# SRainGit/CAE-LO

Measured on AMD Instinct MI355X. Metric: KITTI frames/sec end-to-end (keypts+desc+match+RANSAC), higher is better.
Workload: dtype f32

## Files before the change

cae-lo_amd/csrc/ransac.hip:

```cpp
#include "caelo_internal.h"
#include "caelo_rigid.h"

__device__ inline float residual(const float *R, const float *T, float ax, float ay, float az, float bx, float by, float bz) {
    const float px = __fadd_rn(__fadd_rn(__fadd_rn(__fmul_rn(R[0], bx), __fmul_rn(R[1], by)), __fmul_rn(R[2], bz)), T[0]);
    const float py = __fadd_rn(__fadd_rn(__fadd_rn(__fmul_rn(R[3], bx), __fmul_rn(R[4], by)), __fmul_rn(R[5], bz)), T[1]);
    const float pz = __fadd_rn(__fadd_rn(__fadd_rn(__fmul_rn(R[6], bx), __fmul_rn(R[7], by)), __fmul_rn(R[8], bz)), T[2]);
    const float dx = __fsub_rn(ax, px), dy = __fsub_rn(ay, py), dz = __fsub_rn(az, pz);
    return sqrtf(__fadd_rn(__fadd_rn(__fmul_rn(dx, dx), __fmul_rn(dy, dy)), __fmul_rn(dz, dz)));
}

__global__ void __launch_bounds__(256) k_solve_rt(const float *p0, const float *p1, int n, float *R, float *T, int *credible) {
    __shared__ double red[4][RIGID_TERMS];
    const int tid = threadIdx.x;
    RigidSums sums;
    for (int i = tid; i < n; i += 256) {
        const float *u = p0 + 3 * (size_t)i, *v = p1 + 3 * (size_t)i;
        sums.add(u[0], u[1], u[2], v[0], v[1], v[2]);
    }
    sums.reduce_wave(red, tid & 63, tid >> 6);
    __syncthreads();
    if (tid == 0) {
        double s[RIGID_TERMS];
        for (int t = 0; t < RIGID_TERMS; ++t) s[t] = RigidSums::combine(red, 4, t);
        const int cred = rigid_from_sums(s, R, T);
// ... 131 lines not shown
    }
#pragma unroll
    for (int i = 0; i < 3; ++i)
#pragma unroll
        for (int j = 0; j < 3; ++j) {
            double h = 0;
#pragma unroll
            for (int q = 0; q < 4; ++q) h += (double)c1[q][i] * (double)c0[q][j];
            H[3 * i + j] = h;
        }
    rigid_from_H<false>(H, m0, m1, R, T);
}

#define RB_G 9.5367431640625e-7f
struct HypBound {
    float a, b;
    int kind;
};
__device__ inline void hypothesis_bound(const Sample4 &s, HypBound &hb) {
    const double *H = s.H;
    const double C0 = H[4] * H[8] - H[5] * H[7], C1 = H[5] * H[6] - H[3] * H[8], C2 = H[3] * H[7] - H[4] * H[6];
    const double C3 = H[2] * H[7] - H[1] * H[8], C4 = H[0] * H[8] - H[2] * H[6], C5 = H[1] * H[6] - H[0] * H[7];
    const double C6 = H[1] * H[5] - H[2] * H[4], C7 = H[2] * H[3] - H[0] * H[5], C8 = H[0] * H[4] - H[1] * H[3];
    const double det = H[0] * C0 + H[1] * C1 + H[2] * C2;
    double I1 = 0.0;
#pragma unroll
    for (int i = 0; i < 9; ++i) I1 += H[i] * H[i];
    const double I2 = C0 * C0 + C1 * C1 + C2 * C2 + C3 * C3 + C4 * C4 + C5 * C5 + C6 * C6 + C7 * C7 + C8 * C8;
    float sumCA = 0.f;
    const float aC[9] = {(float)fabs(C0), (float)fabs(C1), (float)fabs(C2), (float)fabs(C3), (float)fabs(C4), (float)fabs(C5), (float)fabs(C6), (float)fabs(C7), (float)fabs(C8)};
#pragma unroll
    for (int i = 0; i < 3; ++i)
#pragma unroll
        for (int j = 0; j < 3; ++j) {
            float t = 0.f;
#pragma unroll
            for (int q = 0; q < 4; ++q) t += fabsf(s.c1[q][i]) * fabsf(s.c0[q][j]);
            sumCA += aC[3 * i + j] * t;
        }
    hb.kind = 0;
    hb.a = 0.f;
    hb.b = 0.f;
    if (!(I2 > 1e-10 * I1 * I1) || !(I1 > 0.0)) { hb.kind = 2; return; }
    const double kappa = 1.41421356237309515 * I1 / sqrt(I2);
    if (fabs(det) <= 64.0 * 5.9604644775390625e-8 * 1.001 * (double)sumCA) hb.kind = 1;
    if (det * det <= 1e-24 * I1 * I2) hb.kind = 1;
    const double nm0 = sqrt(s.m0[0] * s.m0[0] + s.m0[1] * s.m0[1] + s.m0[2] * s.m0[2]);
    const double nm1 = sqrt(s.m1[0] * s.m1[0] + s.m1[1] * s.m1[1] + s.m1[2] * s.m1[2]);
    hb.a = (float)(1.0001 * (double)RB_G * ((2.0 + kappa) * nm1 + nm0));
    hb.b = (float)(1.0001 * (double)RB_G * (2.0 + kappa));
}

#define RE_WAVES 4
#define RE_LDS_PAIRS 1024

__device__ inline void lane_agreement(const float R[9], const float T[3], int lane, int32_t *faults) {
    if (!faults) return;
    unsigned int diff = 0;
#pragma unroll
    for (int q = 0; q < 9; ++q) diff |= __float_as_uint(R[q]) ^ (unsigned int)__builtin_amdgcn_readfirstlane((int)__float_as_uint(R[q]));
#pragma unroll
    for (int q = 0; q < 3; ++q) diff |= __float_as_uint(T[q]) ^ (unsigned int)__builtin_amdgcn_readfirstlane((int)__float_as_uint(T[q]));
    if (__ballot(diff != 0) != 0ull && lane == 0) atomicAdd(faults, 1);
}

__device__ inline int hypothesis_count(const float *P0, int l0, const int64_t *pidx, const float *P1, int l1, int N, const double *r4,
                                       float thr, int lane, int32_t *faults) {
    float R[9], T[3];
    sample_hypothesis(P0, l0, pidx, P1, l1, N, r4, R, T);
    lane_agreement(R, T, lane, faults);
    int cnt = 0;
    for (int i = lane; i < ((N + 63) & ~63); i += 64) {
        bool in = false;
        if (i < N) {
            const float *a = P0 + (size_t)l0 * (pidx ? pidx[i] : i);
            const float *b = P1 + (size_t)l1 * i;
            in = residual(R, T, a[0], a[1], a[2], b[0], b[1], b[2]) < thr;
        }
        cnt += __popcll(__ballot(in));
    }
    return cnt;
}

#define RH_PER_WAVE 4
template <bool CERT>
__device__ __forceinline__ void four_hypotheses(const float *sP0, const float *sP1, int N, const double *rnd, int trial0, float thr, int lane,
                                       int32_t *faults, int32_t *counts, const float2 *sN = nullptr, caelo_ransac_cert *cert = nullptr,
                                       int level = 0) {
    const int mine = min(trial0 + (lane & (RH_PER_WAVE - 1)), CAELO_RANSAC_MAX_TRIALS - 1);
    float R[9], T[3];
    HypBound hb = {0.f, 0.f, 0};
    if (CERT) {
        Sample4 smp;
        sample4(sP0, 3, nullptr, sP1, 3, N, rnd + (size_t)mine * 4, smp);
        hypothesis_bound(smp, hb);
        if (lane < RH_PER_WAVE && trial0 + lane < CAELO_RANSAC_MAX_TRIALS)
#pragma unroll
            for (int q = 0; q < 4; ++q) (level ? cert->idx_up[level - 1] : cert->idx)[trial0 + lane][q] = smp.idx[q];
        rigid_from_H<false>(smp.H, smp.m0, smp.m1, R, T);
    } else {
        sample_hypothesis(sP0, 3, nullptr, sP1, 3, N, rnd + (size_t)mine * 4, R, T);
    }
    if (faults) {
        unsigned int hsh = 0;
#pragma unroll
        for (int q = 0; q < 9; ++q) hsh = hsh * 0x9E3779B1u + __float_as_uint(R[q]);
#pragma unroll
        for (int q = 0; q < 3; ++q) hsh = hsh * 0x9E3779B1u + __float_as_uint(T[q]);
        const bool bad = hsh != (unsigned int)__shfl_xor((int)hsh, 4) || hsh != (unsigned int)__shfl_xor((int)hsh, 16) ||
                         hsh != (unsigned int)__shfl_xor((int)hsh, 32);
        if (__ballot(bad) != 0ull && lane == 0) atomicAdd(faults, 1);
    }
    float Rs[RH_PER_WAVE][9], Ts[RH_PER_WAVE][3];
#pragma unroll
    for (int h = 0; h < RH_PER_WAVE; ++h) {
#pragma unroll
        for (int q = 0; q < 9; ++q) Rs[h][q] = __int_as_float(__builtin_amdgcn_readlane(__float_as_int(R[q]), h));
#pragma unroll
        for (int q = 0; q < 3; ++q) Ts[h][q] = __int_as_float(__builtin_amdgcn_readlane(__float_as_int(T[q]), h));
    }
    int cnt[RH_PER_WAVE] = {0, 0, 0, 0};
    if (!CERT) {
        for (int i = lane; i < ((N + 63) & ~63); i += 64) {
            const bool live = i < N;
            const int ii = live ? i : 0;
            const float ax = sP0[3 * ii], ay = sP0[3 * ii + 1], az = sP0[3 * ii + 2];
            const float bx = sP1[3 * ii], by = sP1[3 * ii + 1], bz = sP1[3 * ii + 2];
#pragma unroll
            for (int h = 0; h < RH_PER_WAVE; ++h) {
                const bool in = live && residual(Rs[h], Ts[h], ax, ay, az, bx, by, bz) < thr;
                cnt[h] += __popcll(__ballot(in));
            }
        }
    } else {
        float as[RH_PER_WAVE], bs[RH_PER_WAVE];
        int kinds[RH_PER_WAVE];
#pragma unroll
        for (int h = 0; h < RH_PER_WAVE; ++h) {
            as[h] = thr + __int_as_float(__builtin_amdgcn_readlane(__float_as_int(hb.a), h));
            bs[h] = __int_as_float(__builtin_amdgcn_readlane(__float_as_int(hb.b), h));
            kinds[h] = __builtin_amdgcn_readlane(hb.kind, h);
        }
        int hi[RH_PER_WAVE] = {0, 0, 0, 0};
        for (int i = lane; i < ((N + 63) & ~63); i += 64) {
            const bool live = i < N;
            const int ii = live ? i : 0;
            const float ax = sP0[3 * ii], ay = sP0[3 * ii + 1], az = sP0[3 * ii + 2];
            const float bx = sP1[3 * ii], by = sP1[3 * ii + 1], bz = sP1[3 * ii + 2];
            const float2 nn = sN[ii];
#pragma unroll
            for (int h = 0; h < RH_PER_WAVE; ++h) {
                const float r = residual(Rs[h], Ts[h], ax, ay, az, bx, by, bz);
                cnt[h] += __popcll(__ballot(live && r < thr));
                hi[h] += __popcll(__ballot(live && r < as[h] + fmaf(bs[h], nn.x, nn.y)));
            }
        }
        if ((kinds[0] | kinds[1] | kinds[2] | kinds[3]) & 1) {
            float Ra[9], Ta[3], Rb[9], Tb[3];
            bool two;
            {
                Sample4 smp;
                sample4(sP0, 3, nullptr, sP1, 3, N, rnd + (size_t)mine * 4, smp);
                two = rigid_two_candidates(smp.H, smp.m0, smp.m1, Ra, Ta, Rb, Tb);
            }
            int ha[RH_PER_WAVE] = {0, 0, 0, 0};
#pragma unroll 1
            for (int h = 0; h < RH_PER_WAVE; ++h) {
                if (kinds[h] != 1) continue;
                if (!__builtin_amdgcn_readlane((int)two, h)) { ha[h] = N; continue; }
                float Ras[9], Tas[3], Rbs[9], Tbs[3];
#pragma unroll
                for (int q = 0; q < 9; ++q) {
                    Ras[q] = __int_as_float(__builtin_amdgcn_readlane(__float_as_int(Ra[q]), h));
                    Rbs[q] = __int_as_float(__builtin_amdgcn_readlane(__float_as_int(Rb[q]), h));
                }
#pragma unroll
                for (int q = 0; q < 3; ++q) {
                    Tas[q] = __int_as_float(__builtin_amdgcn_readlane(__float_as_int(Ta[q]), h));
                    Tbs[q] = __int_as_float(__builtin_amdgcn_readlane(__float_as_int(Tb[q]), h));
                }
                int na = 0, nb = 0;
                for (int i = lane; i < ((N + 63) & ~63); i += 64) {
                    const bool live = i < N;
                    const int ii = live ? i : 0;
                    const float ax = sP0[3 * ii], ay = sP0[3 * ii + 1], az = sP0[3 * ii + 2];
                    const float bx = sP1[3 * ii], by = sP1[3 * ii + 1], bz = sP1[3 * ii + 2];
                    const float2 nn = sN[ii];
                    const float lim = as[h] + fmaf(bs[h], nn.x, nn.y);
                    na += __popcll(__ballot(live && residual(Ras, Tas, ax, ay, az, bx, by, bz) < lim));
                    nb += __popcll(__ballot(live && residual(Rbs, Tbs, ax, ay, az, bx, by, bz) < lim));
                }
                ha[h] = max(na, nb);
            }
#pragma unroll
            for (int h = 0; h < RH_PER_WAVE; ++h)
                if (kinds[h] == 1) hi[h] = max(hi[h], ha[h]);
        }
#pragma unroll
        for (int h = 0; h < RH_PER_WAVE; ++h)
            if (kinds[h] == 2) hi[h] = N;
        if (lane < RH_PER_WAVE && trial0 + lane < CAELO_RANSAC_MAX_TRIALS)
            (level ? cert->hi_up[level - 1] : cert->hi)[trial0 + lane] = lane == 0 ? hi[0] : (lane == 1 ? hi[1] : (lane == 2 ? hi[2] : hi[3]));
    }
    if (lane < RH_PER_WAVE && trial0 + lane < CAELO_RANSAC_MAX_TRIALS)
        counts[trial0 + lane] = lane == 0 ? cnt[0] : (lane == 1 ? cnt[1] : (lane == 2 ? cnt[2] : cnt[3]));
}

template <class PS>
static __device__ __forceinline__ void ransac_hyp_body(const PS &ps, int ld0, int ld1, int64_t k1_max) {
    const auto &P = pair_of(ps, blockIdx.z);
    const float *__restrict__ pc0 = P.pc0, *__restrict__ pc1 = P.pc1;
    const int64_t *__restrict__ pair_idx = P.pair_idx;
    RansacWs *ws = (RansacWs *)P.ws_ransac;
    __shared__ float sP0[RE_LDS_PAIRS * 3], sP1[RE_LDS_PAIRS * 3];
    __shared__ float2 sN[RE_LDS_PAIRS];
    caelo_ransac_cert *cert = P.cert;
    const int N = (P.n0 && *P.n0 <= 0) ? 0 : (P.n1 ? min(max(*P.n1, 0), (int)k1_max) : (int)k1_max);
    const int tid = threadIdx.x, lane = tid & 63, wave = tid >> 6;
    const bool in_lds = N <= RE_LDS_PAIRS;
    if (in_lds) {
        for (int i = tid; i < N; i += 64 * RE_WAVES) {
            const float *a = pc0 + (size_t)ld0 * pair_idx[i];
            const float *b = pc1 + (size_t)ld1 * i;
            const float a0 = a[0], a1 = a[1], a2 = a[2], b0 = b[0], b1 = b[1], b2 = b[2];
            sP0[3 * i] = a0; sP0[3 * i + 1] = a1; sP0[3 * i + 2] = a2;
            sP1[3 * i] = b0; sP1[3 * i + 1] = b1; sP1[3 * i + 2] = b2;
            if (cert) sN[i] = make_float2(1.0001f * sqrtf(b0 * b0 + b1 * b1 + b2 * b2), 1.0001f * RB_G * sqrtf(a0 * a0 + a1 * a1 + a2 * a2));
        }
    }
    __syncthreads();
    if (cert && blockIdx.x == 0 && tid == 0) cert->levels_up = 0;
    if (cert && P.cert_only && blockIdx.x == 0) {
        if (in_lds) {
            float *d0 = &cert->p0[0][0], *d1 = &cert->p1[0][0];
            for (int i = tid; i < 3 * N; i += 64 * RE_WAVES) { d0[i] = sP0[i]; d1[i] = sP1[i]; }
        }
        if (tid == 0) {
            cert->n_pairs = N;
            cert->flags = in_lds ? 0 : CAELO_CERT_NO_BOUNDS;
            cert->magic = CAELO_CERT_MAGIC;
        }
    }
    const int trial0 = (blockIdx.x * RE_WAVES + wave) * RH_PER_WAVE;
    if (trial0 >= CAELO_RANSAC_MAX_TRIALS) return;
    if (!in_lds) {
        for (int h = 0; h < RH_PER_WAVE && trial0 + h < CAELO_RANSAC_MAX_TRIALS; ++h) {
            const int cnt = hypothesis_count(pc0, ld0, pair_idx, pc1, ld1, N, P.rand + (size_t)(trial0 + h) * 4, 0.4f, lane, ps.faults);
            if (lane == 0) ws->counts[trial0 + h] = cnt;
        }
        return;
    }
    if (cert) four_hypotheses<true>(sP0, sP1, N, P.rand, trial0, 0.4f, lane, ps.faults, ws->counts, sN, cert, 0);
    else four_hypotheses<false>(sP0, sP1, N, P.rand, trial0, 0.4f, lane, ps.faults, ws->counts);
}
__global__ void __launch_bounds__(64 * RE_WAVES) k_ransac_hyp(const caelo_pair_set ps, int ld0, int ld1, int64_t k1_max) { ransac_hyp_body(ps, ld0, ld1, k1_max); }
__global__ void __launch_bounds__(64 * RE_WAVES) k_ransac_hyp_tab(const caelo_pair_table pt, int ld0, int ld1, int64_t k1_max) { ransac_hyp_body(pt, ld0, ld1, k1_max); }


#define RU_BLOCKS 32
template <class PS>
static __device__ __forceinline__ void ransac_hyp_up_body(const PS &ps, int ld0, int ld1, int64_t k1_max) {
    const auto &P = pair_of(ps, blockIdx.z);
    caelo_ransac_cert *cert = P.cert;
    if (!cert) return;
    RansacWs *ws = (RansacWs *)P.ws_ransac;
    const int N = (P.n0 && *P.n0 <= 0) ? 0 : (P.n1 ? min(max(*P.n1, 0), (int)k1_max) : (int)k1_max);
    if (N > RE_LDS_PAIRS) return;
    const int least = min(100, (int)(0.2 * (double)N));
    if (least <= 0) return;
    const int tid = threadIdx.x, lane = tid & 63, wave = tid >> 6;
    bool reached = false;
    for (int t = tid; t < CAELO_RANSAC_MAX_TRIALS; t += 64 * RE_WAVES) reached = reached || ws->counts[t] >= least;
    if (__syncthreads_or(reached)) return;
    __shared__ float sP0[RE_LDS_PAIRS * 3], sP1[RE_LDS_PAIRS * 3];
    __shared__ float2 sN[RE_LDS_PAIRS];
    __shared__ int32_t s_scratch[CAELO_RANSAC_MAX_TRIALS];
    const float *__restrict__ pc0 = P.pc0, *__restrict__ pc1 = P.pc1;
    const int64_t *__restrict__ pair_idx = P.pair_idx;
    for (int i = tid; i < N; i += 64 * RE_WAVES) {
        const float *a = pc0 + (size_t)ld0 * pair_idx[i];
        const float *b = pc1 + (size_t)ld1 * i;
        const float a0 = a[0], a1 = a[1], a2 = a[2], b0 = b[0], b1 = b[1], b2 = b[2];
        sP0[3 * i] = a0; sP0[3 * i + 1] = a1; sP0[3 * i + 2] = a2;
        sP1[3 * i] = b0; sP1[3 * i + 1] = b1; sP1[3 * i + 2] = b2;
        sN[i] = make_float2(1.0001f * sqrtf(b0 * b0 + b1 * b1 + b2 * b2), 1.0001f * RB_G * sqrtf(a0 * a0 + a1 * a1 + a2 * a2));
    }
    __syncthreads();
    const int level = 1 + (int)blockIdx.y;
    if (blockIdx.x == 0 && blockIdx.y == 0 && tid == 0) cert->levels_up = 1;
    for (int trial0 = (blockIdx.x * RE_WAVES + wave) * RH_PER_WAVE; trial0 < CAELO_RANSAC_MAX_TRIALS; trial0 += RU_BLOCKS * RE_WAVES * RH_PER_WAVE)
        four_hypotheses<true>(sP0, sP1, N, P.rand + (size_t)level * CAELO_RANSAC_MAX_TRIALS * 4, trial0, 0.4f * (float)(1 << level), lane, ps.faults,
                              s_scratch, sN, cert, level);
}
__global__ void __launch_bounds__(64 * RE_WAVES) k_ransac_hyp_up(const caelo_pair_set ps, int ld0, int ld1, int64_t k1_max) { ransac_hyp_up_body(ps, ld0, ld1, k1_max); }
__global__ void __launch_bounds__(64 * RE_WAVES) k_ransac_hyp_up_tab(const caelo_pair_table pt, int ld0, int ld1, int64_t k1_max) { ransac_hyp_up_body(pt, ld0, ld1, k1_max); }


#define RF_WAVES 8
template <class PS>
static __device__ __forceinline__ void ransac_finish_body(const PS &ps, int ld0, int ld1, int64_t k1_max) {
    const auto &P = pair_of(ps, blockIdx.z);
    if (P.cert && P.cert_only) return;
    const float *__restrict__ pc0 = P.pc0, *__restrict__ pc1 = P.pc1;
    const int64_t *__restrict__ pair_idx = P.pair_idx;
    const double *__restrict__ rnd = P.rand;
    RansacWs *ws = (RansacWs *)P.ws_ransac;
    caelo_pose_result *res = P.result;
    uint8_t *mask = P.mask;
    __shared__ float sP0[RE_LDS_PAIRS * 3], sP1[RE_LDS_PAIRS * 3];
    __shared__ float Rs[9], Ts[3];
    __shared__ RansacVerdict s_v;
    __shared__ double red[4][RIGID_TERMS];
    const int tid = threadIdx.x, lane = tid & 63, wave = tid >> 6;
    const int N = (P.n0 && *P.n0 <= 0) ? 0 : (P.n1 ? min(max(*P.n1, 0), (int)k1_max) : (int)k1_max);
    int c0[(CAELO_RANSAC_MAX_TRIALS + 63) / 64];
    if (wave == 0) {
#pragma unroll
        for (int q = 0; q < (CAELO_RANSAC_MAX_TRIALS + 63) / 64; ++q) {
            const int i = lane * ((CAELO_RANSAC_MAX_TRIALS + 63) / 64) + q;
            c0[q] = i < CAELO_RANSAC_MAX_TRIALS ? ws->counts[i] : 0;
        }
    }
    const bool in_lds = N <= RE_LDS_PAIRS;
    if (in_lds) {
        for (int i = tid; i < N; i += 64 * RF_WAVES) {
            const float *a = pc0 + (size_t)ld0 * pair_idx[i];
            const float *b = pc1 + (size_t)ld1 * i;
            sP0[3 * i] = a[0]; sP0[3 * i + 1] = a[1]; sP0[3 * i + 2] = a[2];
            sP1[3 * i] = b[0]; sP1[3 * i + 1] = b[1]; sP1[3 * i + 2] = b[2];
        }
    }
    if (tid < 64) ransac_replay(N, ws->counts, &s_v, c0);
    __syncthreads();
    if (P.cert) {
        caelo_ransac_cert *cert = P.cert;
        if (in_lds) {
            float *d0 = &cert->p0[0][0], *d1 = &cert->p1[0][0];
            for (int i = tid; i < 3 * N; i += 64 * RF_WAVES) { d0[i] = sP0[i]; d1[i] = sP1[i]; }
        }
        if (tid == 0) {
            cert->n_pairs = N;
            cert->flags = in_lds ? 0 : CAELO_CERT_NO_BOUNDS;
            cert->magic = CAELO_CERT_MAGIC;
        }
    }
    int level = 0;
    while (!s_v.success && level < CAELO_RANSAC_LEVELS - 1) {
        __syncthreads();
        ++level;
        const float thr_l = 0.4f * (float)(1 << level);
        const double *rnd_l = rnd + (size_t)level * CAELO_RANSAC_MAX_TRIALS * 4;
        if (in_lds) {
            for (int trial0 = wave * RH_PER_WAVE; trial0 < CAELO_RANSAC_MAX_TRIALS; trial0 += RF_WAVES * RH_PER_WAVE)
                four_hypotheses<false>(sP0, sP1, N, rnd_l, trial0, thr_l, lane, ps.faults, ws->counts);
        } else {
            for (int trial = wave; trial < CAELO_RANSAC_MAX_TRIALS; trial += RF_WAVES) {
                const int cnt = hypothesis_count(pc0, ld0, pair_idx, pc1, ld1, N, rnd_l + (size_t)trial * 4, thr_l, lane, ps.faults);
                if (lane == 0) ws->counts[trial] = cnt;
            }
        }
        __threadfence_block();
        __syncthreads();
        if (tid < 64) ransac_replay(N, ws->counts, &s_v);
        __syncthreads();
    }
    const int success = s_v.success, best = s_v.best_trial;
    const float thr = 0.4f * (float)(1 << level);
    if (tid < 64) {
        float R[9] = {1.f, 0.f, 0.f, 0.f, 1.f, 0.f, 0.f, 0.f, 1.f}, T[3] = {0.f, 0.f, 0.f};
        if (best >= 0) {
            const double *r4 = rnd + ((size_t)level * CAELO_RANSAC_MAX_TRIALS + best) * 4;
            if (in_lds) sample_hypothesis(sP0, 3, nullptr, sP1, 3, N, r4, R, T);
            else sample_hypothesis(pc0, ld0, pair_idx, pc1, ld1, N, r4, R, T);
        }
        lane_agreement(R, T, lane, ps.faults);
        if (tid < 9) Rs[tid] = R[tid];
        if (tid < 3) Ts[tid] = T[tid];
    }
    __syncthreads();
    double acc[RIGID_TERMS];
#pragma unroll
    for (int t = 0; t < RIGID_TERMS; ++t) acc[t] = 0.0;
    const bool word_ok = (((uintptr_t)mask) & 3u) == 0;
    for (int i0 = tid * 4; tid < 256 && i0 < (int)k1_max; i0 += 4 * 256) {
        unsigned int packed = 0;
#pragma unroll
        for (int q = 0; q < 4; ++q) {
            const int i = i0 + q;
            if (i < N && best >= 0) {
                const float *a = in_lds ? sP0 + 3 * i : pc0 + (size_t)ld0 * pair_idx[i];
                const float *b = in_lds ? sP1 + 3 * i : pc1 + (size_t)ld1 * i;
                const float ax = a[0], ay = a[1], az = a[2], bx = b[0], by = b[1], bz = b[2];
                if (residual(Rs, Ts, ax, ay, az, bx, by, bz) < thr) {
                    packed |= 1u << (8 * q);
                    const double x0 = ax, y0 = ay, z0 = az, x1 = bx, y1 = by, z1 = bz;
                    acc[0] += 1.0;
                    acc[1] += x0; acc[2] += y0; acc[3] += z0;
                    acc[4] += x1; acc[5] += y1; acc[6] += z1;
                    acc[7] += x1 * x0; acc[8] += x1 * y0; acc[9] += x1 * z0;
                    acc[10] += y1 * x0; acc[11] += y1 * y0; acc[12] += y1 * z0;
                    acc[13] += z1 * x0; acc[14] += z1 * y0; acc[15] += z1 * z0;
                }
            }
        }
        if (word_ok && i0 + 3 < (int)k1_max) *(unsigned int *)(mask + i0) = packed;
        else
            for (int q = 0; q < 4 && i0 + q < (int)k1_max; ++q) mask[i0 + q] = (uint8_t)((packed >> (8 * q)) & 1u);
    }
#pragma unroll
    for (int t = 0; t < RIGID_TERMS; ++t)
#pragma unroll
        for (int o = 32; o > 0; o >>= 1) acc[t] += __shfl_xor(acc[t], o);
    if (lane == 0 && wave < 4)
#pragma unroll
        for (int t = 0; t < RIGID_TERMS; ++t) red[wave][t] = acc[t];
    __syncthreads();
    if (tid < 9) { res->R_ransac[tid] = Rs[tid]; }
    if (tid < 3) { res->T_ransac[tid] = Ts[tid]; }
    if (tid == 0) {
        double sm[RIGID_TERMS];
#pragma unroll
        for (int t = 0; t < RIGID_TERMS; ++t) sm[t] = ((red[0][t] + red[1][t]) + red[2][t]) + red[3][t];
        const int n_in = (int)sm[0];
        res->threshold = thr;
        res->success = success;
        res->iterations = s_v.iterations;
        res->n_inliers = n_in;
        res->best_trial = best >= 0 ? level * CAELO_RANSAC_MAX_TRIALS + best : -1;
        res->n_pairs = N;
        float R[9], T[3];
#pragma unroll
        for (int q = 0; q < 9; ++q) R[q] = Rs[q];
#pragma unroll
        for (int q = 0; q < 3; ++q) T[q] = Ts[q];
        if (n_in > 0) {
            const double cnt = sm[0];
            const double m0[3] = {sm[1] / cnt, sm[2] / cnt, sm[3] / cnt}, m1[3] = {sm[4] / cnt, sm[5] / cnt, sm[6] / cnt};
            double H[9];
#pragma unroll
            for (int i = 0; i < 3; ++i)
#pragma unroll
                for (int j = 0; j < 3; ++j) H[3 * i + j] = sm[7 + 3 * i + j] - cnt * m1[i] * m0[j];
            rigid_from_H(H, m0, m1, R, T);
        }
#pragma unroll
        for (int q = 0; q < 9; ++q) res->R[q] = R[q];
#pragma unroll
        for (int q = 0; q < 3; ++q) res->T[q] = T[q];
    }
}
__global__ void __launch_bounds__(64 * RF_WAVES, 4) k_ransac_finish(const caelo_pair_set ps, int ld0, int ld1, int64_t k1_max) { ransac_finish_body(ps, ld0, ld1, k1_max); }
__global__ void __launch_bounds__(64 * RF_WAVES, 4) k_ransac_finish_tab(const caelo_pair_table pt, int ld0, int ld1, int64_t k1_max) { ransac_finish_body(pt, ld0, ld1, k1_max); }


CAELO_API int caelo_ransac(caelo_ctx *c, const float *pc0, int ld0, const float *pc1, int ld1, const int64_t *pair_idx,
                           int64_t k1_max, const int32_t *n1, const double *rnd, caelo_pose_result *result,
                           uint8_t *inlier_mask, void *wsv, caelo_ransac_cert *cert, void *stream) {
    CAELO_REQUIRE(c && pc0 && pc1 && pair_idx && rnd && result && inlier_mask && wsv, "null argument");
    CAELO_REQUIRE((((uintptr_t)cert) & 15u) == 0, "certificate not 16-byte aligned");
    caelo_pair_set ps = {};
    ps.n = 1;
    ps.faults = c->faults;
    caelo_pair_dev &p = ps.p[0];
    p.pc0 = pc0; p.pc1 = pc1; p.pair_idx = const_cast<int64_t *>(pair_idx); p.n1 = n1; p.rand = rnd; p.result = result;
    p.mask = inlier_mask; p.ws_ransac = wsv; p.cert = cert;
    return ransac_set(ps, ld0, ld1, k1_max, caelo_stream(stream));
}

template <class PS>
static int ransac_launch(const PS &ps, int ld0, int ld1, int64_t k1_max, bool any_cert, bool all_cert_only, hipStream_t s,
                         void (*hyp)(PS, int, int, int64_t), void (*hyp_up)(PS, int, int, int64_t), void (*finish)(PS, int, int, int64_t)) {
    hyp<<<dim3((CAELO_RANSAC_MAX_TRIALS + RE_WAVES * RH_PER_WAVE - 1) / (RE_WAVES * RH_PER_WAVE), 1, ps.n), 64 * RE_WAVES, 0, s>>>(ps, ld0, ld1, k1_max);
    CAELO_LAUNCH_CHECK();
    if (any_cert) {
        hyp_up<<<dim3(RU_BLOCKS, 2, ps.n), 64 * RE_WAVES, 0, s>>>(ps, ld0, ld1, k1_max);
        CAELO_LAUNCH_CHECK();
    }
    if (all_cert_only) return CAELO_OK;
    finish<<<dim3(1, 1, ps.n), 64 * RF_WAVES, 0, s>>>(ps, ld0, ld1, k1_max);
    CAELO_LAUNCH_CHECK();
    return CAELO_OK;
}

int ransac_set(const caelo_pair_set &ps, int ld0, int ld1, int64_t k1_max, hipStream_t s) {
    CAELO_REQUIRE(ps.n >= 1 && ps.n <= CAELO_FB_MAX, "bad pair count");
    CAELO_REQUIRE(k1_max > 0 && ld0 >= 3 && ld1 >= 3, "bad shape");
    bool any_cert = false, all_cert_only = true;
    for (int i = 0; i < ps.n; ++i) {
        any_cert = any_cert || ps.p[i].cert != nullptr;
        all_cert_only = all_cert_only && ps.p[i].cert && ps.p[i].cert_only;
    }
    return ransac_launch(ps, ld0, ld1, k1_max, any_cert, all_cert_only, s, k_ransac_hyp, k_ransac_hyp_up, k_ransac_finish);
}

int ransac_table(const caelo_pair_table &pt, hipStream_t s) {
    CAELO_REQUIRE(pt.n >= 1 && pt.n <= CAELO_FB_MAX, "bad pair count");
    return ransac_launch(pt, 64, 64, CAELO_MAX_KEYPTS, pt.cert != nullptr, pt.cert && pt.cert_only, s, k_ransac_hyp_tab, k_ransac_hyp_up_tab,
                         k_ransac_finish_tab);
}
```

cae-lo_amd/csrc/ring.hip:

```cpp
#include <math.h>
#include <stdarg.h>

#include <vector>

#include "caelo_internal.h"

static thread_local char g_err[512] = "";

void caelo_set_error(const char *fmt, ...) {
    va_list ap;
    va_start(ap, fmt);
    vsnprintf(g_err, sizeof(g_err), fmt, ap);
    va_end(ap);
}

CAELO_API const char *caelo_last_error(void) { return g_err; }
CAELO_API int caelo_abi_version(void) { return CAELO_ABI_VERSION; }
#ifndef CAELO_BUILD_WORD
#define CAELO_BUILD_WORD 0
#endif
CAELO_API int caelo_build_flags(void) { return CAELO_BUILD_WORD; }

static int proj_edge_table(double **out);

// ... 173 lines not shown
        const int n0 = CAELO_RING_W - c0 < 64 ? CAELO_RING_W - c0 : 64;
        const int in0 = CAELO_NET_W - c0 < n0 ? (CAELO_NET_W - c0 > 0 ? CAELO_NET_W - c0 : 0) : n0;
        const unsigned long long E0 = in0 < 64 ? E & ((1ull << in0) - 1ull) : E;
        const unsigned long long E1 = n0 < 64 && r0 + 1 < CAELO_NET_H ? E >> n0 : 0ull;
        const int b0 = c0 >> 5, l1 = 32 - (c0 & 31);
        const unsigned long long rest = E0 >> l1;
        const unsigned int hit0 = __builtin_amdgcn_readfirstlane((E0 & ((1ull << l1) - 1ull)) != 0ull ? 1u : 0u) |
                                  __builtin_amdgcn_readfirstlane((unsigned int)rest != 0u ? 2u : 0u) |
                                  __builtin_amdgcn_readfirstlane((unsigned int)(rest >> 32) != 0u ? 4u : 0u);
        const unsigned int hit1 = __builtin_amdgcn_readfirstlane((unsigned int)E1 != 0u ? 1u : 0u) |
                                  __builtin_amdgcn_readfirstlane((unsigned int)(E1 >> 32) != 0u ? 2u : 0u);
        if ((threadIdx.x & 63) == 0) {
            if (hit0) atomicOr(&s_rows[r0 - rw], (unsigned long long)hit0 << b0);
            if (hit1) atomicOr(&s_rows[1], (unsigned long long)hit1);
        }
    }
    caelo_lds_barrier();
    if (threadIdx.x < 2 && s_rows[threadIdx.x] != 0ull) atomicOr(&kmap[rw + threadIdx.x], s_rows[threadIdx.x]);
}

static int64_t set_max_points(const caelo_frame_set &fs) {
    int64_t n = 0;
    for (int i = 0; i < fs.n; ++i) n = fs.f[i].n > n ? fs.f[i].n : n;
    return n;
}

int ring_project_launch(caelo_ctx *c, const float *pc, int64_t n, float *ring, int32_t *counter, int32_t *winner_ws, int32_t *status,
                        hipStream_t s) {
    caelo_frame_set fs = {};
    fs.n = 1;
    fs.f[0].pc = pc; fs.f[0].n = n; fs.f[0].ring = ring; fs.f[0].counter = counter; fs.f[0].winner = winner_ws; fs.f[0].status = status;
    return ring_project_set(c, fs, s);
}

int ring_project_set(caelo_ctx *c, const caelo_frame_set &fs, hipStream_t s) {
    const int npix = CAELO_RING_H * CAELO_RING_W;
    const int64_t n = set_max_points(fs);
    const ProjConst k = proj_const(c->proj_edge);
    k_project_points<<<dim3((unsigned)((n + 255) / 256), 1, fs.n), 256, 0, s>>>(fs, k);
    CAELO_LAUNCH_CHECK();
    k_ring_fill<<<dim3((npix + 255) / 256, 1, fs.n), 256, 0, s>>>(fs);
    CAELO_LAUNCH_CHECK();
    return CAELO_OK;
}

CAELO_API int caelo_project(caelo_ctx *c, const float *pc, int64_t n, float *ring, int32_t *counter,
                            int32_t *winner_ws, int32_t *status, void *stream) {
    CAELO_REQUIRE(c && pc && ring && counter && winner_ws && status, "null argument");
    CAELO_REQUIRE(n > 3, "PC.shape[0] > 3 (SphericalRing.py:73)");
    hipStream_t s = caelo_stream(stream);
    const size_t npix = CAELO_RING_H * CAELO_RING_W;
    caelo_clear_list cl;
    cl.n = 0;
    cl.item[cl.n++] = {winner_ws, npix * sizeof(int32_t), 0xFFFFFFFFu};
    cl.item[cl.n++] = {counter, npix * sizeof(int32_t), 0u};
    int rc = caelo_clear_many(cl, s);
    if (rc) return rc;
    return ring_project_launch(c, pc, n, ring, counter, winner_ws, status, s);
}


#define RESP_PT 2
#define RESP_BPX (16 * RESP_PT)
#define RESP_ROW ((RESP_BPX + 2) * 3)
#define RESP_STAGE (3 * RESP_ROW)
typedef float resp_f4 __attribute__((ext_vector_type(4)));

static void respond_fragments(const float *w1, const float *b1, const float *w2, const float *b2, float *out) {
    for (int lane = 0; lane < 64; ++lane) {
        const int g = lane >> 4, n = lane & 15;
        int f = 0;
        for (int t = 0; t < 2; ++t)
            for (int s = 0; s < 7; ++s) {
                const int k = 4 * s + g;
                out[(f++) * 64 + lane] = k < 27 ? w1[k * 32 + 16 * t + 4 * (n & 3) + (n >> 2)] : 0.0f;
            }
        for (int t = 0; t < 2; ++t)
            for (int r = 0; r < 4; ++r) out[(f++) * 64 + lane] = b1[16 * t + 4 * r + g];
        for (int s = 0; s < 8; ++s) out[(f++) * 64 + lane] = n < 8 ? w2[(4 * s + g) * 8 + n] : 0.0f;
        for (int r = 0; r < 4; ++r) out[(f++) * 64 + lane] = g < 2 ? b2[4 * g + r] : 0.0f;
    }
}

__global__ void __launch_bounds__(64) k_respond_mfma(const caelo_frame_set fs, int in_w, int in_c, const float *__restrict__ wts, int row0) {
    const float *__restrict__ in = fs.f[blockIdx.z].ring;
    float *__restrict__ resp = fs.f[blockIdx.z].resp;
    const int lane = threadIdx.x, g = lane >> 4, n = lane & 15;
    const int y = blockIdx.y + row0;
    constexpr int NBLK = CAELO_NET_W / RESP_BPX, NLD = (RESP_STAGE + 63) / 64;
    static_assert(NBLK <= 64 && CAELO_NET_H <= 64, "one map word per row, one bit per block");
    unsigned long long todo = 0ull;
    for (int b = blockIdx.x; b < NBLK; b += gridDim.x) todo |= 1ull << b;
    if (const unsigned long long *__restrict__ kmap = fs.f[blockIdx.z].kp_elig) {
        unsigned long long m = 0ull;
#pragma unroll
        for (int dy = -2; dy <= 2; ++dy) m |= (unsigned)(y + dy) < (unsigned)CAELO_NET_H ? kmap[y + dy] : 0ull;
        todo &= m | m << 1 | m >> 1;
    }
    if (todo == 0ull) return;
    __shared__ float s_in[2][((RESP_STAGE + 63) / 64) * 64];
    int goff[NLD];
    unsigned int edge = 0u;
    float v[NLD];
#pragma unroll
    for (int q = 0; q < NLD; ++q) {
        const int i = lane + 64 * q;
        const int row = i / RESP_ROW, j = i - row * RESP_ROW, px = j / 3, ci = j - px * 3;
        const int yy = y + row - 1;
        const bool ok = i < RESP_STAGE && (unsigned)yy < (unsigned)CAELO_NET_H;
        goff[q] = ok ? (yy * in_w + px - 1) * in_c + ci : -1;
        edge |= (px == 0 ? 1u : 0u) << q | (px == RESP_BPX + 1 ? 1u : 0u) << (16 + q);
    }
    const __amdgpu_buffer_rsrc_t rsrc = __builtin_amdgcn_make_buffer_rsrc((void *)in, 0, CAELO_NET_H * in_w * in_c * 4, 0x00020000);
#define RESP_LOAD(BLK)                                                                                            \
    _Pragma("unroll") for (int q = 0; q < NLD; ++q) {                                                              \
        const unsigned int hide = ((BLK) == 0 ? edge : 0u) | ((BLK) == NBLK - 1 ? edge >> 16 : 0u);               \
        const bool ok_ = goff[q] >= 0 && !((hide >> q) & 1u);                                                     \
        const int ob_ = ok_ ? (goff[q] + (BLK) * RESP_BPX * in_c) * 4 : 0x7FFFFFF0;                               \
        v[q] = __builtin_bit_cast(float, __builtin_amdgcn_raw_buffer_load_b32(rsrc, ob_, 0, 0));                  \
    }
#define RESP_STORE(BUF)                                                                                           \
    _Pragma("unroll") for (int q = 0; q < NLD; ++q) s_in[BUF][lane + 64 * q] = v[q];
    int blk = __builtin_ctzll(todo), buf = 0;
    todo &= todo - 1ull;
    RESP_LOAD(blk)
    const float *fr = wts + RESP_FRAG_OFF + lane;
    float a1[2][7], a2[8];
    resp_f4 c1[2], c2;
#pragma unroll
    for (int t = 0; t < 2; ++t)
#pragma unroll
        for (int s = 0; s < 7; ++s) a1[t][s] = fr[(t * 7 + s) * 64];
#pragma unroll
    for (int t = 0; t < 2; ++t)
#pragma unroll
        for (int r = 0; r < 4; ++r) c1[t][r] = fr[(14 + t * 4 + r) * 64];
#pragma unroll
    for (int s = 0; s < 8; ++s) a2[s] = fr[(22 + s) * 64];
#pragma unroll
    for (int r = 0; r < 4; ++r) c2[r] = fr[(30 + r) * 64];
    int loff[7];
#pragma unroll
    for (int s = 0; s < 7; ++s) {
        const int k = 4 * s + g;
        const int kc = k < 27 ? k : 26;
        const int ky = kc / 9, kx = (kc / 3) % 3, ci = kc % 3;
        loff[s] = ky * RESP_ROW + (n + kx) * 3 + ci;
    }
#pragma unroll
    for (int t = 0; t < 2; ++t) {
#pragma unroll
        for (int s = 0; s < 7; ++s) __asm__ volatile("" : "+v"(a1[t][s]));
        __asm__ volatile("" : "+v"(c1[t]));
    }
#pragma unroll
    for (int s = 0; s < 8; ++s) __asm__ volatile("" : "+v"(a2[s]));
    __asm__ volatile("" : "+v"(c2));
    RESP_STORE(0)
    for (;; buf ^= 1) {
        const bool more = todo != 0ull;
        const int next = more ? __builtin_ctzll(todo) : 0;
        todo &= todo - 1ull;
        if (more) RESP_LOAD(next)
        __builtin_amdgcn_fence(__ATOMIC_RELEASE, "wavefront");
        __builtin_amdgcn_wave_barrier();
        __builtin_amdgcn_fence(__ATOMIC_ACQUIRE, "wavefront");
        float b[RESP_PT][7];
#pragma unroll
        for (int pt = 0; pt < RESP_PT; ++pt)
#pragma unroll
            for (int s = 0; s < 7; ++s) b[pt][s] = s_in[buf][loff[s] + 48 * pt];
        __builtin_amdgcn_sched_barrier(0);
        resp_f4 h[RESP_PT][2], o[RESP_PT];
#pragma unroll
        for (int pt = 0; pt < RESP_PT; ++pt) { h[pt][0] = c1[0]; h[pt][1] = c1[1]; o[pt] = c2; }
#pragma unroll
        for (int s = 0; s < 7; ++s)
#pragma unroll
            for (int pt = 0; pt < RESP_PT; ++pt)
#pragma unroll
                for (int t = 0; t < 2; ++t) h[pt][t] = __builtin_amdgcn_mfma_f32_16x16x4f32(a1[t][s], b[pt][s], h[pt][t], 0, 0, 0);
#pragma unroll
        for (int t = 0; t < 2; ++t)
#pragma unroll
            for (int r = 0; r < 4; ++r)
#pragma unroll
                for (int pt = 0; pt < RESP_PT; ++pt) {
                    const float hv = h[pt][t][r] > 0.0f ? h[pt][t][r] : 0.0f;
                    o[pt] = __builtin_amdgcn_mfma_f32_16x16x4f32(a2[4 * t + r], hv, o[pt], 0, 0, 0);
                }
        if (g < 2) {
#pragma unroll
            for (int pt = 0; pt < RESP_PT; ++pt) {
                const int x = blk * RESP_BPX + 16 * pt + n;
                *(float4 *)(resp + ((int64_t)y * CAELO_NET_W + x) * 8 + 4 * g) =
                    make_float4(o[pt][0] > 0.0f ? o[pt][0] : 0.0f, o[pt][1] > 0.0f ? o[pt][1] : 0.0f, o[pt][2] > 0.0f ? o[pt][2] : 0.0f,
                                o[pt][3] > 0.0f ? o[pt][3] : 0.0f);
            }
        }
        if (!more) break;
// ... 487 lines not shown
```

Baseline: 19090.

## Give each RANSAC wave sixteen hypotheses when batches are large; tune respond occupancy

Generalizes the four-hypothesis-per-wave scoring into a templated per-wave count, processed in passes of four, and uses sixteen hypotheses per wave (fewer blocks) when the pair batch has at least four pairs. The finish kernel always uses the wide variant. This amortizes per-hypothesis sampling across more lanes and cuts launch width, at the cost of longer serial work per wave. Separately, the respond MFMA kernel gets a waves-per-EU hint and a sentinel change that fixes left-edge offsets that were negative but valid.

```diff
diff --git a/cae-lo_amd/csrc/ransac.hip b/cae-lo_amd/csrc/ransac.hip
--- a/cae-lo_amd/csrc/ransac.hip
+++ b/cae-lo_amd/csrc/ransac.hip
@@ -237,19 +237,24 @@
     return cnt;
 }
 
-#define RH_PER_WAVE 4
-template <bool CERT>
-__device__ __forceinline__ void four_hypotheses(const float *sP0, const float *sP1, int N, const double *rnd, int trial0, float thr, int lane,
+#define RH_WIDE 16
+#define RH_NARROW 4
+#define RH_WIDE_FROM 4
+#define RH_PER_PASS 4
+#define RH_BLOCKS(PW) ((CAELO_RANSAC_MAX_TRIALS + RE_WAVES * (PW) - 1) / (RE_WAVES * (PW)))
+template <bool CERT, int PW>
+__device__ __forceinline__ void wave_hypotheses(const float *sP0, const float *sP1, int N, const double *rnd, int trial0, float thr, int lane,
                                        int32_t *faults, int32_t *counts, const float2 *sN = nullptr, caelo_ransac_cert *cert = nullptr,
                                        int level = 0) {
-    const int mine = min(trial0 + (lane & (RH_PER_WAVE - 1)), CAELO_RANSAC_MAX_TRIALS - 1);
+    const int mine = min(trial0 + (lane & (PW - 1)), CAELO_RANSAC_MAX_TRIALS - 1);
+    const bool stores = lane < PW && trial0 + lane < CAELO_RANSAC_MAX_TRIALS;
     float R[9], T[3];
     HypBound hb = {0.f, 0.f, 0};
     if (CERT) {
         Sample4 smp;
         sample4(sP0, 3, nullptr, sP1, 3, N, rnd + (size_t)mine * 4, smp);
         hypothesis_bound(smp, hb);
-        if (lane < RH_PER_WAVE && trial0 + lane < CAELO_RANSAC_MAX_TRIALS)
+        if (stores)
 #pragma unroll
             for (int q = 0; q < 4; ++q) (level ? cert->idx_up[level - 1] : cert->idx)[trial0 + lane][q] = smp.idx[q];
         rigid_from_H<false>(smp.H, smp.m0, smp.m1, R, T);
@@ -262,55 +267,63 @@
         for (int q = 0; q < 9; ++q) hsh = hsh * 0x9E3779B1u + __float_as_uint(R[q]);
 #pragma unroll
         for (int q = 0; q < 3; ++q) hsh = hsh * 0x9E3779B1u + __float_as_uint(T[q]);
-        const bool bad = hsh != (unsigned int)__shfl_xor((int)hsh, 4) || hsh != (unsigned int)__shfl_xor((int)hsh, 16) ||
-                         hsh != (unsigned int)__shfl_xor((int)hsh, 32);
+        bool bad = false;
+#pragma unroll
+        for (int o = PW; o < 64; o <<= 1) bad = bad || hsh != (unsigned int)__shfl_xor((int)hsh, o);
         if (__ballot(bad) != 0ull && lane == 0) atomicAdd(faults, 1);
     }
-    float Rs[RH_PER_WAVE][9], Ts[RH_PER_WAVE][3];
-#pragma unroll
-    for (int h = 0; h < RH_PER_WAVE; ++h) {
-#pragma unroll
-        for (int q = 0; q < 9; ++q) Rs[h][q] = __int_as_float(__builtin_amdgcn_readlane(__float_as_int(R[q]), h));
-#pragma unroll
-        for (int q = 0; q < 3; ++q) Ts[h][q] = __int_as_float(__builtin_amdgcn_readlane(__float_as_int(T[q]), h));
-    }
-    int cnt[RH_PER_WAVE] = {0, 0, 0, 0};
-    if (!CERT) {
-        for (int i = lane; i < ((N + 63) & ~63); i += 64) {
-            const bool live = i < N;
-            const int ii = live ? i : 0;
-            const float ax = sP0[3 * ii], ay = sP0[3 * ii + 1], az = sP0[3 * ii + 2];
-            const float bx = sP1[3 * ii], by = sP1[3 * ii + 1], bz = sP1[3 * ii + 2];
-#pragma unroll
-            for (int h = 0; h < RH_PER_WAVE; ++h) {
-                const bool in = live && residual(Rs[h], Ts[h], ax, ay, az, bx, by, bz) < thr;
-                cnt[h] += __popcll(__ballot(in));
+    int my_cnt = 0, my_hi = 0;
+#pragma unroll 1
+    for (int l0 = 0; l0 < PW && trial0 + l0 < CAELO_RANSAC_MAX_TRIALS; l0 += RH_PER_PASS) {
+        float Rs[RH_PER_PASS][9], Ts[RH_PER_PASS][3];
+#pragma unroll
+        for (int h = 0; h < RH_PER_PASS; ++h) {
+#pragma unroll
+            for (int q = 0; q < 9; ++q) Rs[h][q] = __int_as_float(__builtin_amdgcn_readlane(__float_as_int(R[q]), l0 + h));
+#pragma unroll
+            for (int q = 0; q < 3; ++q) Ts[h][q] = __int_as_float(__builtin_amdgcn_readlane(__float_as_int(T[q]), l0 + h));
+        }
+        int cnt[RH_PER_PASS] = {0, 0, 0, 0};
+        const int hh = lane - l0;
+        if (!CERT) {
+            for (int i = lane; i < ((N + 63) & ~63); i += 64) {
+                const bool live = i < N;
+                const int ii = live ? i : 0;
+                const float ax = sP0[3 * ii], ay = sP0[3 * ii + 1], az = sP0[3 * ii + 2];
+                const float bx = sP1[3 * ii], by = sP1[3 * ii + 1], bz = sP1[3 * ii + 2];
+#pragma unroll
+                for (int h = 0; h < RH_PER_PASS; ++h) {
+                    const bool in = live && residual(Rs[h], Ts[h], ax, ay, az, bx, by, bz) < thr;
+                    cnt[h] += __popcll(__ballot(in));
+                }
             }
-        }
-    } else {
-        float as[RH_PER_WAVE], bs[RH_PER_WAVE];
-        int kinds[RH_PER_WAVE];
-#pragma unroll
-        for (int h = 0; h < RH_PER_WAVE; ++h) {
-            as[h] = thr + __int_as_float(__builtin_amdgcn_readlane(__float_as_int(hb.a), h));
-            bs[h] = __int_as_float(__builtin_amdgcn_readlane(__float_as_int(hb.b), h));
-            kinds[h] = __builtin_amdgcn_readlane(hb.kind, h);
-        }
-        int hi[RH_PER_WAVE] = {0, 0, 0, 0};
-        for (int i = lane; i < ((N + 63) & ~63); i += 64) {
-            const bool live = i < N;
-            const int ii = live ? i : 0;
-            const float ax = sP0[3 * ii], ay = sP0[3 * ii + 1], az = sP0[3 * ii + 2];
-            const float bx = sP1[3 * ii], by = sP1[3 * ii + 1], bz = sP1[3 * ii + 2];
-            const float2 nn = sN[ii];
-#pragma unroll
-            for (int h = 0; h < RH_PER_WAVE; ++h) {
-                const float r = residual(Rs[h], Ts[h], ax, ay, az, bx, by, bz);
-                cnt[h] += __popcll(__ballot(live && r < thr));
-                hi[h] += __popcll(__ballot(live && r < as[h] + fmaf(bs[h], nn.x, nn.y)));
+        } else {
+            float as[RH_PER_PASS], bs[RH_PER_PASS];
+#pragma unroll
+            for (int h = 0; h < RH_PER_PASS; ++h) {
+                as[h] = thr + __int_as_float(__builtin_amdgcn_readlane(__float_as_int(hb.a), l0 + h));
+                bs[h] = __int_as_float(__builtin_amdgcn_readlane(__float_as_int(hb.b), l0 + h));
             }
-        }
-        if ((kinds[0] | kinds[1] | kinds[2] | kinds[3]) & 1) {
+            int hi[RH_PER_PASS] = {0, 0, 0, 0};
+            for (int i = lane; i < ((N + 63) & ~63); i += 64) {
+                const bool live = i < N;
+                const int ii = live ? i : 0;
+                const float ax = sP0[3 * ii], ay = sP0[3 * ii + 1], az = sP0[3 * ii + 2];
+                const float bx = sP1[3 * ii], by = sP1[3 * ii + 1], bz = sP1[3 * ii + 2];
+                const float2 nn = sN[ii];
+#pragma unroll
+                for (int h = 0; h < RH_PER_PASS; ++h) {
+                    const float r = residual(Rs[h], Ts[h], ax, ay, az, bx, by, bz);
+                    cnt[h] += __popcll(__ballot(live && r < thr));
+                    hi[h] += __popcll(__ballot(live && r < as[h] + fmaf(bs[h], nn.x, nn.y)));
+                }
+            }
+            if (hh >= 0 && hh < RH_PER_PASS) my_hi = hh == 0 ? hi[0] : (hh == 1 ? hi[1] : (hh == 2 ? hi[2] : hi[3]));
+        }
+        if (hh >= 0 && hh < RH_PER_PASS) my_cnt = hh == 0 ? cnt[0] : (hh == 1 ? cnt[1] : (hh == 2 ? cnt[2] : cnt[3]));
+    }
+    if (CERT) {
+        if (__ballot(stores && hb.kind == 1) != 0ull) {
             float Ra[9], Ta[3], Rb[9], Tb[3];
             bool two;
             {
@@ -318,50 +331,47 @@
                 sample4(sP0, 3, nullptr, sP1, 3, N, rnd + (size_t)mine * 4, smp);
                 two = rigid_two_candidates(smp.H, smp.m0, smp.m1, Ra, Ta, Rb, Tb);
             }
-            int ha[RH_PER_WAVE] = {0, 0, 0, 0};
 #pragma unroll 1
-            for (int h = 0; h < RH_PER_WAVE; ++h) {
-                if (kinds[h] != 1) continue;
-                if (!__builtin_amdgcn_readlane((int)two, h)) { ha[h] = N; continue; }
-                float Ras[9], Tas[3], Rbs[9], Tbs[3];
-#pragma unroll
-                for (int q = 0; q < 9; ++q) {
-                    Ras[q] = __int_as_float(__builtin_amdgcn_readlane(__float_as_int(Ra[q]), h));
-                    Rbs[q] = __int_as_float(__builtin_amdgcn_readlane(__float_as_int(Rb[q]), h));
+            for (int h = 0; h < PW && trial0 + h < CAELO_RANSAC_MAX_TRIALS; ++h) {
+                if (__builtin_amdgcn_readlane(hb.kind, h) != 1) continue;
+                int ha = N;
+                if (__builtin_amdgcn_readlane((int)two, h)) {
+                    const float as = thr + __int_as_float(__builtin_amdgcn_readlane(__float_as_int(hb.a), h));
+                    const float bs = __int_as_float(__builtin_amdgcn_readlane(__float_as_int(hb.b), h));
+                    float Ras[9], Tas[3], Rbs[9], Tbs[3];
+#pragma unroll
+                    for (int q = 0; q < 9; ++q) {
+                        Ras[q] = __int_as_float(__builtin_amdgcn_readlane(__float_as_int(Ra[q]), h));
+                        Rbs[q] = __int_as_float(__builtin_amdgcn_readlane(__float_as_int(Rb[q]), h));
+                    }
+#pragma unroll
+                    for (int q = 0; q < 3; ++q) {
+                        Tas[q] = __int_as_float(__builtin_amdgcn_readlane(__float_as_int(Ta[q]), h));
+                        Tbs[q] = __int_as_float(__builtin_amdgcn_readlane(__float_as_int(Tb[q]), h));
+                    }
+                    int na = 0, nb = 0;
+                    for (int i = lane; i < ((N + 63) & ~63); i += 64) {
+                        const bool live = i < N;
+                        const int ii = live ? i : 0;
+                        const float ax = sP0[3 * ii], ay = sP0[3 * ii + 1], az = sP0[3 * ii + 2];
+                        const float bx = sP1[3 * ii], by = sP1[3 * ii + 1], bz = sP1[3 * ii + 2];
+                        const float2 nn = sN[ii];
+                        const float lim = as + fmaf(bs, nn.x, nn.y);
+                        na += __popcll(__ballot(live && residual(Ras, Tas, ax, ay, az, bx, by, bz) < lim));
+                        nb += __popcll(__ballot(live && residual(Rbs, Tbs, ax, ay, az, bx, by, bz) < lim));
+                    }
+                    ha = max(na, nb);
                 }
-#pragma unroll
-                for (int q = 0; q < 3; ++q) {
-                    Tas[q] = __int_as_float(__builtin_amdgcn_readlane(__float_as_int(Ta[q]), h));
-                    Tbs[q] = __int_as_float(__builtin_amdgcn_readlane(__float_as_int(Tb[q]), h));
-                }
-                int na = 0, nb = 0;
-                for (int i = lane; i < ((N + 63) & ~63); i += 64) {
-                    const bool live = i < N;
-                    const int ii = live ? i : 0;
-                    const float ax = sP0[3 * ii], ay = sP0[3 * ii + 1], az = sP0[3 * ii + 2];
-                    const float bx = sP1[3 * ii], by = sP1[3 * ii + 1], bz = sP1[3 * ii + 2];
-                    const float2 nn = sN[ii];
-                    const float lim = as[h] + fmaf(bs[h], nn.x, nn.y);
-                    na += __popcll(__ballot(live && residual(Ras, Tas, ax, ay, az, bx, by, bz) < lim));
-                    nb += __popcll(__ballot(live && residual(Rbs, Tbs, ax, ay, az, bx, by, bz) < lim));
-                }
-                ha[h] = max(na, nb);
+                if (lane == h) my_hi = max(my_hi, ha);
             }
-#pragma unroll
-            for (int h = 0; h < RH_PER_WAVE; ++h)
-                if (kinds[h] == 1) hi[h] = max(hi[h], ha[h]);
-        }
-#pragma unroll
-        for (int h = 0; h < RH_PER_WAVE; ++h)
-            if (kinds[h] == 2) hi[h] = N;
-        if (lane < RH_PER_WAVE && trial0 + lane < CAELO_RANSAC_MAX_TRIALS)
-            (level ? cert->hi_up[level - 1] : cert->hi)[trial0 + lane] = lane == 0 ? hi[0] : (lane == 1 ? hi[1] : (lane == 2 ? hi[2] : hi[3]));
-    }
-    if (lane < RH_PER_WAVE && trial0 + lane < CAELO_RANSAC_MAX_TRIALS)
-        counts[trial0 + lane] = lane == 0 ? cnt[0] : (lane == 1 ? cnt[1] : (lane == 2 ? cnt[2] : cnt[3]));
-}
-
-template <class PS>
+        }
+        if (hb.kind == 2) my_hi = N;
+        if (stores) (level ? cert->hi_up[level - 1] : cert->hi)[trial0 + lane] = my_hi;
+    }
+    if (stores) counts[trial0 + lane] = my_cnt;
+}
+
+template <int PW, class PS>
 static __device__ __forceinline__ void ransac_hyp_body(const PS &ps, int ld0, int ld1, int64_t k1_max) {
     const auto &P = pair_of(ps, blockIdx.z);
     const float *__restrict__ pc0 = P.pc0, *__restrict__ pc1 = P.pc1;
@@ -396,24 +406,23 @@
             cert->magic = CAELO_CERT_MAGIC;
         }
     }
-    const int trial0 = (blockIdx.x * RE_WAVES + wave) * RH_PER_WAVE;
+    const int trial0 = (blockIdx.x * RE_WAVES + wave) * PW;
     if (trial0 >= CAELO_RANSAC_MAX_TRIALS) return;
     if (!in_lds) {
-        for (int h = 0; h < RH_PER_WAVE && trial0 + h < CAELO_RANSAC_MAX_TRIALS; ++h) {
+        for (int h = 0; h < PW && trial0 + h < CAELO_RANSAC_MAX_TRIALS; ++h) {
             const int cnt = hypothesis_count(pc0, ld0, pair_idx, pc1, ld1, N, P.rand + (size_t)(trial0 + h) * 4, 0.4f, lane, ps.faults);
             if (lane == 0) ws->counts[trial0 + h] = cnt;
         }
         return;
     }
-    if (cert) four_hypotheses<true>(sP0, sP1, N, P.rand, trial0, 0.4f, lane, ps.faults, ws->counts, sN, cert, 0);
-    else four_hypotheses<false>(sP0, sP1, N, P.rand, trial0, 0.4f, lane, ps.faults, ws->counts);
-}
-__global__ void __launch_bounds__(64 * RE_WAVES) k_ransac_hyp(const caelo_pair_set ps, int ld0, int ld1, int64_t k1_max) { ransac_hyp_body(ps, ld0, ld1, k1_max); }
-__global__ void __launch_bounds__(64 * RE_WAVES) k_ransac_hyp_tab(const caelo_pair_table pt, int ld0, int ld1, int64_t k1_max) { ransac_hyp_body(pt, ld0, ld1, k1_max); }
-
-
-#define RU_BLOCKS 32
-template <class PS>
+    if (cert) wave_hypotheses<true, PW>(sP0, sP1, N, P.rand, trial0, 0.4f, lane, ps.faults, ws->counts, sN, cert, 0);
+    else wave_hypotheses<false, PW>(sP0, sP1, N, P.rand, trial0, 0.4f, lane, ps.faults, ws->counts);
+}
+template <int PW> __global__ void __launch_bounds__(64 * RE_WAVES) k_ransac_hyp(const caelo_pair_set ps, int ld0, int ld1, int64_t k1_max) { ransac_hyp_body<PW>(ps, ld0, ld1, k1_max); }
+template <int PW> __global__ void __launch_bounds__(64 * RE_WAVES) k_ransac_hyp_tab(const caelo_pair_table pt, int ld0, int ld1, int64_t k1_max) { ransac_hyp_body<PW>(pt, ld0, ld1, k1_max); }
+
+
+template <int PW, class PS>
 static __device__ __forceinline__ void ransac_hyp_up_body(const PS &ps, int ld0, int ld1, int64_t k1_max) {
     const auto &P = pair_of(ps, blockIdx.z);
     caelo_ransac_cert *cert = P.cert;
@@ -443,12 +452,12 @@
     __syncthreads();
     const int level = 1 + (int)blockIdx.y;
     if (blockIdx.x == 0 && blockIdx.y == 0 && tid == 0) cert->levels_up = 1;
-    for (int trial0 = (blockIdx.x * RE_WAVES + wave) * RH_PER_WAVE; trial0 < CAELO_RANSAC_MAX_TRIALS; trial0 += RU_BLOCKS * RE_WAVES * RH_PER_WAVE)
-        four_hypotheses<true>(sP0, sP1, N, P.rand + (size_t)level * CAELO_RANSAC_MAX_TRIALS * 4, trial0, 0.4f * (float)(1 << level), lane, ps.faults,
+    for (int trial0 = (blockIdx.x * RE_WAVES + wave) * PW; trial0 < CAELO_RANSAC_MAX_TRIALS; trial0 += RH_BLOCKS(PW) * RE_WAVES * PW)
+        wave_hypotheses<true, PW>(sP0, sP1, N, P.rand + (size_t)level * CAELO_RANSAC_MAX_TRIALS * 4, trial0, 0.4f * (float)(1 << level), lane, ps.faults,
                               s_scratch, sN, cert, level);
 }
-__global__ void __launch_bounds__(64 * RE_WAVES) k_ransac_hyp_up(const caelo_pair_set ps, int ld0, int ld1, int64_t k1_max) { ransac_hyp_up_body(ps, ld0, ld1, k1_max); }
-__global__ void __launch_bounds__(64 * RE_WAVES) k_ransac_hyp_up_tab(const caelo_pair_table pt, int ld0, int ld1, int64_t k1_max) { ransac_hyp_up_body(pt, ld0, ld1, k1_max); }
+template <int PW> __global__ void __launch_bounds__(64 * RE_WAVES) k_ransac_hyp_up(const caelo_pair_set ps, int ld0, int ld1, int64_t k1_max) { ransac_hyp_up_body<PW>(ps, ld0, ld1, k1_max); }
+template <int PW> __global__ void __launch_bounds__(64 * RE_WAVES) k_ransac_hyp_up_tab(const caelo_pair_table pt, int ld0, int ld1, int64_t k1_max) { ransac_hyp_up_body<PW>(pt, ld0, ld1, k1_max); }
 
 
 #define RF_WAVES 8
@@ -506,8 +515,8 @@
         const float thr_l = 0.4f * (float)(1 << level);
         const double *rnd_l = rnd + (size_t)level * CAELO_RANSAC_MAX_TRIALS * 4;
         if (in_lds) {
-            for (int trial0 = wave * RH_PER_WAVE; trial0 < CAELO_RANSAC_MAX_TRIALS; trial0 += RF_WAVES * RH_PER_WAVE)
-                four_hypotheses<false>(sP0, sP1, N, rnd_l, trial0, thr_l, lane, ps.faults, ws->counts);
+            for (int trial0 = wave * RH_WIDE; trial0 < CAELO_RANSAC_MAX_TRIALS; trial0 += RF_WAVES * RH_WIDE)
+                wave_hypotheses<false, RH_WIDE>(sP0, sP1, N, rnd_l, trial0, thr_l, lane, ps.faults, ws->counts);
         } else {
             for (int trial = wave; trial < CAELO_RANSAC_MAX_TRIALS; trial += RF_WAVES) {
                 const int cnt = hypothesis_count(pc0, ld0, pair_idx, pc1, ld1, N, rnd_l + (size_t)trial * 4, thr_l, lane, ps.faults);
@@ -623,12 +632,12 @@
 }
 
 template <class PS>
-static int ransac_launch(const PS &ps, int ld0, int ld1, int64_t k1_max, bool any_cert, bool all_cert_only, hipStream_t s,
+static int ransac_launch(const PS &ps, int ld0, int ld1, int64_t k1_max, bool any_cert, bool all_cert_only, hipStream_t s, int per_wave,
                          void (*hyp)(PS, int, int, int64_t), void (*hyp_up)(PS, int, int, int64_t), void (*finish)(PS, int, int, int64_t)) {
-    hyp<<<dim3((CAELO_RANSAC_MAX_TRIALS + RE_WAVES * RH_PER_WAVE - 1) / (RE_WAVES * RH_PER_WAVE), 1, ps.n), 64 * RE_WAVES, 0, s>>>(ps, ld0, ld1, k1_max);
+    hyp<<<dim3(RH_BLOCKS(per_wave), 1, ps.n), 64 * RE_WAVES, 0, s>>>(ps, ld0, ld1, k1_max);
     CAELO_LAUNCH_CHECK();
     if (any_cert) {
-        hyp_up<<<dim3(RU_BLOCKS, 2, ps.n), 64 * RE_WAVES, 0, s>>>(ps, ld0, ld1, k1_max);
+        hyp_up<<<dim3(RH_BLOCKS(per_wave), 2, ps.n), 64 * RE_WAVES, 0, s>>>(ps, ld0, ld1, k1_max);
         CAELO_LAUNCH_CHECK();
     }
     if (all_cert_only) return CAELO_OK;
@@ -645,11 +654,17 @@
         any_cert = any_cert || ps.p[i].cert != nullptr;
         all_cert_only = all_cert_only && ps.p[i].cert && ps.p[i].cert_only;
     }
-    return ransac_launch(ps, ld0, ld1, k1_max, any_cert, all_cert_only, s, k_ransac_hyp, k_ransac_hyp_up, k_ransac_finish);
+    if (ps.n >= RH_WIDE_FROM)
+        return ransac_launch(ps, ld0, ld1, k1_max, any_cert, all_cert_only, s, RH_WIDE, k_ransac_hyp<RH_WIDE>, k_ransac_hyp_up<RH_WIDE>, k_ransac_finish);
+    return ransac_launch(ps, ld0, ld1, k1_max, any_cert, all_cert_only, s, RH_NARROW, k_ransac_hyp<RH_NARROW>, k_ransac_hyp_up<RH_NARROW>, k_ransac_finish);
 }
 
 int ransac_table(const caelo_pair_table &pt, hipStream_t s) {
     CAELO_REQUIRE(pt.n >= 1 && pt.n <= CAELO_FB_MAX, "bad pair count");
-    return ransac_launch(pt, 64, 64, CAELO_MAX_KEYPTS, pt.cert != nullptr, pt.cert && pt.cert_only, s, k_ransac_hyp_tab, k_ransac_hyp_up_tab,
+    const bool any_cert = pt.cert != nullptr, all_cert_only = pt.cert && pt.cert_only;
+    if (pt.n >= RH_WIDE_FROM)
+        return ransac_launch(pt, 64, 64, CAELO_MAX_KEYPTS, any_cert, all_cert_only, s, RH_WIDE, k_ransac_hyp_tab<RH_WIDE>, k_ransac_hyp_up_tab<RH_WIDE>,
+                             k_ransac_finish_tab);
+    return ransac_launch(pt, 64, 64, CAELO_MAX_KEYPTS, any_cert, all_cert_only, s, RH_NARROW, k_ransac_hyp_tab<RH_NARROW>, k_ransac_hyp_up_tab<RH_NARROW>,
                          k_ransac_finish_tab);
 }
diff --git a/cae-lo_amd/csrc/ring.hip b/cae-lo_amd/csrc/ring.hip
--- a/cae-lo_amd/csrc/ring.hip
+++ b/cae-lo_amd/csrc/ring.hip
@@ -279,7 +279,8 @@
     }
 }
 
-__global__ void __launch_bounds__(64) k_respond_mfma(const caelo_frame_set fs, int in_w, int in_c, const float *__restrict__ wts, int row0) {
+__global__ void __launch_bounds__(64) __attribute__((amdgpu_waves_per_eu(5, 5)))
+k_respond_mfma(const caelo_frame_set fs, int in_w, int in_c, const float *__restrict__ wts, int row0) {
     const float *__restrict__ in = fs.f[blockIdx.z].ring;
     float *__restrict__ resp = fs.f[blockIdx.z].resp;
     const int lane = threadIdx.x, g = lane >> 4, n = lane & 15;
@@ -296,6 +297,7 @@
     }
     if (todo == 0ull) return;
     __shared__ float s_in[2][((RESP_STAGE + 63) / 64) * 64];
+    constexpr int RESP_NO_ELEMENT = -0x40000000;
     int goff[NLD];
     unsigned int edge = 0u;
     float v[NLD];
@@ -305,14 +307,14 @@
         const int row = i / RESP_ROW, j = i - row * RESP_ROW, px = j / 3, ci = j - px * 3;
         const int yy = y + row - 1;
         const bool ok = i < RESP_STAGE && (unsigned)yy < (unsigned)CAELO_NET_H;
-        goff[q] = ok ? (yy * in_w + px - 1) * in_c + ci : -1;
+        goff[q] = ok ? (yy * in_w + px - 1) * in_c + ci : RESP_NO_ELEMENT;
         edge |= (px == 0 ? 1u : 0u) << q | (px == RESP_BPX + 1 ? 1u : 0u) << (16 + q);
     }
     const __amdgpu_buffer_rsrc_t rsrc = __builtin_amdgcn_make_buffer_rsrc((void *)in, 0, CAELO_NET_H * in_w * in_c * 4, 0x00020000);
 #define RESP_LOAD(BLK)                                                                                            \
     _Pragma("unroll") for (int q = 0; q < NLD; ++q) {                                                              \
         const unsigned int hide = ((BLK) == 0 ? edge : 0u) | ((BLK) == NBLK - 1 ? edge >> 16 : 0u);               \
-        const bool ok_ = goff[q] >= 0 && !((hide >> q) & 1u);                                                     \
+        const bool ok_ = goff[q] != RESP_NO_ELEMENT && !((hide >> q) & 1u);                                       \
         const int ob_ = ok_ ? (goff[q] + (BLK) * RESP_BPX * in_c) * 4 : 0x7FFFFFF0;                               \
         v[q] = __builtin_bit_cast(float, __builtin_amdgcn_raw_buffer_load_b32(rsrc, ob_, 0, 0));                  \
     }
```

After: 19340, median of 6. 1.3% higher.
